# EasyVision-Ton/VMG

Hardware: AMD Instinct MI355X
Metric: LR-frames/s (train: forward+loss+backward+AdamW), VMG-REDS-few_levels 4x SR (higher is better)
Workload: dtype bf16; 1 GPU; VMG-REDS-few_levels train step, per-GPU batch 4x7x3x64x64 -> 4x SR (BASELINE configs[1]); global_batch=4, frames_per_clip=7, parallelism=dp1, launch=eager, recompute_chains=False, fp8_chains=False

## Files before the change

vmg_amd/csrc/ltam.hip:

```cpp
#include "common.h"

namespace {

constexpr int LT_TILE = 8;
constexpr int LT_PIX = 64;
constexpr int LT_HEADS = 4;
constexpr int LT_MAX_T = 32;

struct LtamK {
  const char* q;
  const char* k[LT_MAX_T];
  const char* v[LT_MAX_T];
  const float* loc;
  const float* rpe;
  const float* decay;
  char* out;
  float* lse;
  const char* dout;
  char* dq;
  void* dk_acc[LT_MAX_T];
  void* dv_acc[LT_MAX_T];
  float* drpe;
  int n, h, w, c, t, wh, ww;
  float scale;
  int tiles_x, tiles_y;
  int dbg;
};

__device__ __forceinline__ int nearest_index(float lx, float ly, int w, int h) {
  const float dx = (float)(w - 1 > 1 ? w - 1 : 1), dy = (float)(h - 1 > 1 ? h - 1 : 1);
  const float gx = __fsub_rn(__fdiv_rn(__fmul_rn(2.0f, lx), dx), 1.0f);
  const float gy = __fsub_rn(__fdiv_rn(__fmul_rn(2.0f, ly), dy), 1.0f);
  const float ix = __fmul_rn(__fdiv_rn(__fadd_rn(gx, 1.0f), 2.0f), (float)(w - 1));
  const float iy = __fmul_rn(__fdiv_rn(__fadd_rn(gy, 1.0f), 2.0f), (float)(h - 1));
  const float xn = nearbyintf(ix), yn = nearbyintf(iy);
  if (!(xn >= 0.f && xn <= (float)(w - 1) && yn >= 0.f && yn <= (float)(h - 1))) return -1;
  return (int)yn * w + (int)xn;
}

__device__ __forceinline__ float quad_sum(float v) {
  v += __shfl_xor(v, 1, 64);
  v += __shfl_xor(v, 2, 64);
  return v;
}

typedef __attribute__((ext_vector_type(4))) unsigned int lt_u32x4;
__device__ __attribute__((aligned(16))) unsigned int g_ltam_zero[4] = {0, 0, 0, 0};

template <typename T, int D>
struct RowCopy {
  static constexpr int VN = 16 / sizeof(T), NVEC = LT_HEADS * D / VN, TOTAL = LT_PIX * NVEC, NIT = (TOTAL + 255) / 256;
  lt_u32x4 r[NIT];
  __device__ __forceinline__ void fetch(const T* src_base, const int* src_idx, int tid) {
    constexpr int c = LT_HEADS * D;
#pragma unroll
    for (int k = 0; k < NIT; ++k) {
      const int i = tid + k * 256;
      const int p = min(i / NVEC, LT_PIX - 1), v = i - (i / NVEC) * NVEC;
      const int s_ = src_idx[p];
      const bool ok = i < TOTAL && s_ >= 0;
      const T* src = ok ? src_base + (long long)s_ * c + v * VN : reinterpret_cast<const T*>(g_ltam_zero);
      r[k] = *reinterpret_cast<const lt_u32x4*>(src);
    }
  }
  __device__ __forceinline__ void store(T* dst, int row_stride, int tid) const {
#pragma unroll
    for (int k = 0; k < NIT; ++k) {
      const int i = tid + k * 256;
      const int p = i / NVEC, v = i - p * NVEC;
      if (i < TOTAL) *reinterpret_cast<lt_u32x4*>(dst + p * row_stride + v * VN) = r[k];
    }
  }
};

template <typename T, int D>
__device__ __forceinline__ void load_slice(const T* p, float (&o)[D]) {
  static_assert(D % 4 == 0, "head dim must be a multiple of 4");
  if constexpr (sizeof(T) == 2) {
#pragma unroll
    for (int i = 0; i < D / 4; ++i) {
      const bf16x4 t = *reinterpret_cast<const bf16x4*>(reinterpret_cast<const bf16*>(p) + 4 * i);
#pragma unroll
      for (int e = 0; e < 4; ++e) o[4 * i + e] = (float)t[e];
    }
  } else {
#pragma unroll
    for (int i = 0; i < D / 4; ++i) {
      const f32x4 t = *reinterpret_cast<const f32x4*>(reinterpret_cast<const float*>(p) + 4 * i);
#pragma unroll
      for (int e = 0; e < 4; ++e) o[4 * i + e] = t[e];
    }
  }
}

template <typename T, int D>
__global__ __launch_bounds__(256) void ltam_fwd_kernel(const LtamK a) {
  extern __shared__ __attribute__((aligned(16))) char smem[];
  constexpr int c = LT_HEADS * D, RS = c + 16 / sizeof(T);
  T* qt = reinterpret_cast<T*>(smem);
  T* kt = qt + LT_PIX * RS;
  T* vt = kt + LT_PIX * RS;
  float* knorm = reinterpret_cast<float*>(vt + LT_PIX * RS);
  int* sidx = reinterpret_cast<int*>(knorm + LT_PIX);
  int* selfidx = sidx + LT_PIX;

  const int tid = threadIdx.x, p = tid >> 2, hd = tid & 3;
  const int tyi = p >> 3, txi = p & 7;
  int bid = blockIdx.x;
  const int tx = bid % a.tiles_x;
  bid /= a.tiles_x;
  const int ty = bid % a.tiles_y, n = bid / a.tiles_y;
  const int y = ty * LT_TILE + tyi, x = tx * LT_TILE + txi;
  const bool inside = y < a.h && x < a.w;
  const long long img = (long long)n * a.h * a.w;
  if (tid < LT_PIX) {
    const int yy = ty * LT_TILE + (tid >> 3), xx = tx * LT_TILE + (tid & 7);
    selfidx[tid] = (yy < a.h && xx < a.w) ? yy * a.w + xx : -1;
  }
  __syncthreads();
  RowCopy<T, D> rk, rv;
  rk.fetch(reinterpret_cast<const T*>(a.q) + img * c, selfidx, tid);
  rk.store(qt, RS, tid);
  __syncthreads();
  float qs[D];
  float ss = 0.f;
  load_slice<T, D>(qt + p * RS + hd * D, qs);
#pragma unroll
  for (int d = 0; d < D; ++d) ss += qs[d] * qs[d];
  {
    const float inv = a.scale / fmaxf(sqrtf(quad_sum(ss)), 1e-12f);
#pragma unroll
    for (int d = 0; d < D; ++d) qs[d] *= inv;
  }
  const int wq = a.wh * a.ww;
  const int wy0 = (tyi / a.wh) * a.wh, wx0 = (txi / a.ww) * a.ww;
  const int qi = (tyi - wy0) * a.ww + (txi - wx0);
  const float dec = a.decay[hd];
  float m = -INFINITY, l = 0.f, acc[D];
#pragma unroll
  for (int d = 0; d < D; ++d) acc[d] = 0.f;

  for (int j = 0; j < a.t; ++j) {
    __syncthreads();
    if (tid < LT_PIX) {
      int s = -1;
      if (selfidx[tid] >= 0) {
        const long long lb = ((long long)n * 2 * a.t + 2 * j) * a.h * a.w + selfidx[tid];
        s = nearest_index(a.loc[lb], a.loc[lb + (long long)a.h * a.w], a.w, a.h);
      }
      sidx[tid] = s;
    }
    __syncthreads();
    rk.fetch(reinterpret_cast<const T*>(a.k[j]) + img * c, sidx, tid);
    rv.fetch(reinterpret_cast<const T*>(a.v[j]) + img * c, sidx, tid);
    rk.store(kt, RS, tid);
    rv.store(vt, RS, tid);
    __syncthreads();
    {
      float s2 = 0.f, kv[D];
      load_slice<T, D>(kt + p * RS + hd * D, kv);
#pragma unroll
      for (int d = 0; d < D; ++d) s2 += kv[d] * kv[d];
      s2 = quad_sum(s2);
      if (hd == 0) knorm[p] = fmaxf(sqrtf(s2), 1e-12f);
    }
    __syncthreads();
    float pw = dec;
    for (int e = 1; e < a.t - j; ++e) pw *= dec;
    for (int ki = 0; ki < wq; ++ki) {
      const int pk = (wy0 + ki / a.ww) * LT_TILE + wx0 + ki % a.ww;
      float dot = 0.f, kk[D], vv[D];
      load_slice<T, D>(kt + pk * RS + hd * D, kk);
      load_slice<T, D>(vt + pk * RS + hd * D, vv);
#pragma unroll
      for (int d = 0; d < D; ++d) dot += qs[d] * kk[d];
      const float logit = dot / knorm[pk] + pw * a.rpe[(hd * wq + qi) * wq + ki];
      const float mn = fmaxf(m, logit);
      const float corr = __expf(m - mn), pe = __expf(logit - mn);
      l = l * corr + pe;
#pragma unroll
      for (int d = 0; d < D; ++d) acc[d] = acc[d] * corr + pe * vv[d];
      m = mn;
    }
  }
  if (inside) {
    const float inv = 1.f / l;
    T* o = reinterpret_cast<T*>(a.out) + (img + (long long)y * a.w + x) * c + hd * D;
#pragma unroll
    for (int d = 0; d < D; ++d) o[d] = from_f32<T>(acc[d] * inv);
    if (a.lse) a.lse[(img + (long long)y * a.w + x) * LT_HEADS + hd] = m + __logf(l);
  }
}

template <int C>
__device__ __forceinline__ void scatter_rows(void* acc, long long img, const float* rowbuf, const int* sidx, const int* selfidx, int tid, bool skip) {
  float* dst = reinterpret_cast<float*>(acc);
  for (int i = tid; i < LT_PIX * C; i += 256) {
    const int pp = i / C, ch = i - pp * C;
    const int sp = sidx[pp];
    if (sp >= 0 && selfidx[pp] >= 0 && !skip) atomicAdd(dst + (img + sp) * C + ch, rowbuf[i]);
  }
}

#ifdef VMG_DIAG
#define LT_ABL(bit) (a.dbg & (bit))
#else
#define LT_ABL(bit) false
#endif
template <typename T, int D>
__global__ __launch_bounds__(256) void ltam_bwd_kernel(const LtamK a) {
  extern __shared__ __attribute__((aligned(16))) char smem[];
  constexpr int c = LT_HEADS * D, RS = c + 16 / sizeof(T);
  T* kt = reinterpret_cast<T*>(smem);
  T* vt = kt + LT_PIX * RS;
  T* dot_ = vt + LT_PIX * RS;
  T* qt = dot_ + LT_PIX * RS;
  float* knorm = reinterpret_cast<float*>(qt + LT_PIX * RS);
  float* qnorm = knorm + LT_PIX;
  float* lse = qnorm + LT_PIX;
  float* delta = lse + LT_PIX * LT_HEADS;
  float* drpe_s = delta + LT_PIX * LT_HEADS;
  int* sidx = reinterpret_cast<int*>(drpe_s + LT_HEADS * a.wh * a.ww * a.wh * a.ww);
  int* selfidx = sidx + LT_PIX;

  const int tid = threadIdx.x, p = tid >> 2, hd = tid & 3;
  const int tyi = p >> 3, txi = p & 7;
  int bid = blockIdx.x;
  const int tx = bid % a.tiles_x;
  bid /= a.tiles_x;
  const int ty = bid % a.tiles_y, n = bid / a.tiles_y;
  const int y = ty * LT_TILE + tyi, x = tx * LT_TILE + txi;
  const bool inside = y < a.h && x < a.w;
  const long long img = (long long)n * a.h * a.w;
  const int wq = a.wh * a.ww;
  if (tid < LT_PIX) {
    const int yy = ty * LT_TILE + (tid >> 3), xx = tx * LT_TILE + (tid & 7);
    selfidx[tid] = (yy < a.h && xx < a.w) ? yy * a.w + xx : -1;
  }
  for (int i = tid; i < LT_HEADS * wq * wq; i += 256) drpe_s[i] = 0.f;
  __syncthreads();
  RowCopy<T, D> rk, rv;
  rk.fetch(reinterpret_cast<const T*>(a.dout) + img * c, selfidx, tid);
  rv.fetch(reinterpret_cast<const T*>(a.q) + img * c, selfidx, tid);
  rk.store(dot_, RS, tid);
  rv.store(qt, RS, tid);
  __syncthreads();
  float qn[D], go[D];
  {
    float ss = 0.f, dl = 0.f, ov[D];
    const long long own = (img + (long long)(inside ? y * a.w + x : 0)) * c + hd * D;
    load_slice<T, D>(qt + p * RS + hd * D, qn);
    load_slice<T, D>(dot_ + p * RS + hd * D, go);
    load_slice<T, D>(reinterpret_cast<const T*>(a.out) + own, ov);
#pragma unroll
    for (int d = 0; d < D; ++d) {
      ss += qn[d] * qn[d];
      dl += inside ? go[d] * ov[d] : 0.f;
    }
    const float nr = fmaxf(sqrtf(quad_sum(ss)), 1e-12f);
    if (hd == 0) qnorm[p] = nr;
    const float inv = 1.f / nr;
#pragma unroll
    for (int d = 0; d < D; ++d) qn[d] *= inv;
    delta[p * LT_HEADS + hd] = dl;
    lse[p * LT_HEADS + hd] = inside ? a.lse[(img + (long long)y * a.w + x) * LT_HEADS + hd] : 0.f;
  }
  const int wy0 = (tyi / a.wh) * a.wh, wx0 = (txi / a.ww) * a.ww;
  const int myi = (tyi - wy0) * a.ww + (txi - wx0);
  const float dec = a.decay[hd];
  float dqn[D];
#pragma unroll
  for (int d = 0; d < D; ++d) dqn[d] = 0.f;
  for (int j = 0; j < a.t; ++j) {
    __syncthreads();
    if (tid < LT_PIX) {
      int s = -1;
      if (selfidx[tid] >= 0) {
        const long long lb = ((long long)n * 2 * a.t + 2 * j) * a.h * a.w + selfidx[tid];
        s = nearest_index(a.loc[lb], a.loc[lb + (long long)a.h * a.w], a.w, a.h);
      }
      sidx[tid] = s;
    }
    __syncthreads();
    if (!(LT_ABL(8) && j > 0)) {
      rk.fetch(reinterpret_cast<const T*>(a.k[j]) + img * c, sidx, tid);
      rv.fetch(reinterpret_cast<const T*>(a.v[j]) + img * c, sidx, tid);
    }
    rk.store(kt, RS, tid);
    rv.store(vt, RS, tid);
    __syncthreads();
    float kn[D], vown[D];
    load_slice<T, D>(vt + p * RS + hd * D, vown);
    {
      float s2 = 0.f;
      load_slice<T, D>(kt + p * RS + hd * D, kn);
#pragma unroll
      for (int d = 0; d < D; ++d) s2 += kn[d] * kn[d];
      s2 = quad_sum(s2);
      const float nr = fmaxf(sqrtf(s2), 1e-12f);
      if (hd == 0) knorm[p] = nr;
      const float inv = 1.f / nr;
#pragma unroll
      for (int d = 0; d < D; ++d) kn[d] *= inv;
    }
    __syncthreads();
    float pw = dec;
    for (int e = 1; e < a.t - j; ++e) pw *= dec;

    if (!LT_ABL(4)) {
      const float my_lse = lse[p * LT_HEADS + hd], my_delta = delta[p * LT_HEADS + hd];
      for (int ki = 0; ki < wq; ++ki) {
        const int pk = (wy0 + ki / a.ww) * LT_TILE + wx0 + ki % a.ww;
        const float inv_kn = 1.f / knorm[pk];
        float dot = 0.f, dp = 0.f, kk[D], vv[D];
        load_slice<T, D>(kt + pk * RS + hd * D, kk);
        load_slice<T, D>(vt + pk * RS + hd * D, vv);
#pragma unroll
        for (int d = 0; d < D; ++d) {
          dot += qn[d] * kk[d];
          dp += go[d] * vv[d];
        }
        const float logit = a.scale * dot * inv_kn + pw * a.rpe[(hd * wq + myi) * wq + ki];
        const float pr = __expf(logit - my_lse);
        const float ds = pr * (dp - my_delta);
        if (inside) atomicAdd(&drpe_s[(hd * wq + myi) * wq + ki], ds * pw);
        const float f = ds * a.scale * inv_kn;
#pragma unroll
        for (int d = 0; d < D; ++d) dqn[d] += f * kk[d];
      }
    }
    float dkn[D], dv[D];
#pragma unroll
    for (int d = 0; d < D; ++d) dkn[d] = dv[d] = 0.f;
    for (int qq = 0; qq < wq; ++qq) {
      const int pq = (wy0 + qq / a.ww) * LT_TILE + wx0 + qq % a.ww;
      if (selfidx[pq] < 0 || LT_ABL(2)) continue;
      const float inv_qn = 1.f / qnorm[pq];
      float dot = 0.f, dp = 0.f;
      float qv[D], gg[D];
      load_slice<T, D>(qt + pq * RS + hd * D, qv);
      load_slice<T, D>(dot_ + pq * RS + hd * D, gg);
#pragma unroll
      for (int d = 0; d < D; ++d) {
        qv[d] *= inv_qn;
        dot += qv[d] * kn[d];
        dp += gg[d] * vown[d];
      }
      const float logit = a.scale * dot + pw * a.rpe[(hd * wq + qq) * wq + myi];
      const float pr = __expf(logit - lse[pq * LT_HEADS + hd]);
      const float ds = pr * (dp - delta[pq * LT_HEADS + hd]);
#pragma unroll
      for (int d = 0; d < D; ++d) {
        dkn[d] += ds * a.scale * qv[d];
        dv[d] += pr * gg[d];
      }
    }
    {
      float nd = 0.f;
#pragma unroll
      for (int d = 0; d < D; ++d) nd += kn[d] * dkn[d];
      nd = quad_sum(nd);
      const float inv = 1.f / knorm[p];
      float* rowbuf = reinterpret_cast<float*>(kt);
      __syncthreads();
#pragma unroll
      for (int d = 0; d < D; ++d) rowbuf[p * c + hd * D + d] = (dkn[d] - kn[d] * nd) * inv;
      __syncthreads();
      scatter_rows<c>(a.dk_acc[j], img, rowbuf, sidx, selfidx, tid, LT_ABL(1));
      __syncthreads();
#pragma unroll
      for (int d = 0; d < D; ++d) rowbuf[p * c + hd * D + d] = dv[d];
      __syncthreads();
      scatter_rows<c>(a.dv_acc[j], img, rowbuf, sidx, selfidx, tid, LT_ABL(1));
    }
  }
  {
    float nd = 0.f;
#pragma unroll
    for (int d = 0; d < D; ++d) nd += qn[d] * dqn[d];
    nd = quad_sum(nd);
    if (inside) {
      const float inv = 1.f / qnorm[p];
      T* dq = reinterpret_cast<T*>(a.dq) + (img + (long long)y * a.w + x) * c + hd * D;
#pragma unroll
      for (int d = 0; d < D; ++d) dq[d] = from_f32<T>((dqn[d] - qn[d] * nd) * inv);
    }
  }
  __syncthreads();
  for (int i = tid; i < LT_HEADS * wq * wq; i += 256) atomicAdd(&a.drpe[i], drpe_s[i]);
}

template <typename T, int D>
int launch_ltam(const LtamK& k, bool backward, hipStream_t st) {
  const int RS = k.c + 16 / (int)sizeof(T);
  const int grid = k.n * k.tiles_y * k.tiles_x;
  if (!backward) {
    const int lds = 3 * LT_PIX * RS * (int)sizeof(T) + LT_PIX * 4 + 2 * LT_PIX * 4;
    auto fn = ltam_fwd_kernel<T, D>;
    static bool set[VMG_MAX_DEVICES] = {};
    const int dev = vmg_current_device();
    if (!set[dev]) { (void)hipFuncSetAttribute(reinterpret_cast<const void*>(fn), hipFuncAttributeMaxDynamicSharedMemorySize, 160 * 1024); set[dev] = true; }
    hipLaunchKernelGGL(fn, dim3(grid), dim3(256), lds, st, k);
  } else {
    const int wq = k.wh * k.ww;
    const int lds = 4 * LT_PIX * RS * (int)sizeof(T) + (2 * LT_PIX + 2 * LT_PIX * LT_HEADS + LT_HEADS * wq * wq) * 4 + 2 * LT_PIX * 4;
    VMG_CHECK(lds <= 160 * 1024, "ltam_bwd: LDS request %d B exceeds 160 KiB", lds);
    auto fn = ltam_bwd_kernel<T, D>;
    static bool set[VMG_MAX_DEVICES] = {};
    const int dev = vmg_current_device();
    if (!set[dev]) { (void)hipFuncSetAttribute(reinterpret_cast<const void*>(fn), hipFuncAttributeMaxDynamicSharedMemorySize, 160 * 1024); set[dev] = true; }
    hipLaunchKernelGGL(fn, dim3(grid), dim3(256), lds, st, k);
  }
  VMG_LAUNCH_CHECK();
  return 0;
}

template <typename T>
int dispatch_d(const LtamK& k, bool backward, hipStream_t st) {
  switch (k.c / LT_HEADS) {
    case 4: return launch_ltam<T, 4>(k, backward, st);
    case 8: return launch_ltam<T, 8>(k, backward, st);
    case 28: return launch_ltam<T, 28>(k, backward, st);
    case 36: return launch_ltam<T, 36>(k, backward, st);
  }
  vmg_set_error("ltam: head dim %d not instantiated (supported: 4, 8, 28, 36)", k.c / LT_HEADS);
  return -1;
}

int fill_common(LtamK& k, int dtype, const void* q, const void* const* keys, const void* const* vals, const float* loc, const float* rpe,
                const float* decay, int n, int h, int w, int c, int heads, int wh, int ww, int t, float scale) {
  VMG_CHECK(dtype == VMG_F32 || dtype == VMG_BF16, "ltam: bad dtype");
  VMG_CHECK(q && keys && vals && loc && rpe && decay, "ltam: null pointer");
  VMG_CHECK(heads == LT_HEADS, "ltam: heads must be %d", LT_HEADS);
  VMG_CHECK(t >= 1 && t <= LT_MAX_T, "ltam: 1..%d key-frames", LT_MAX_T);
  VMG_CHECK(n > 0 && h > 0 && w > 0 && c % (LT_HEADS * (dtype == VMG_BF16 ? 8 : 4) / LT_HEADS) == 0 && c % LT_HEADS == 0, "ltam: bad shape");
  VMG_CHECK(wh >= 1 && ww >= 1 && LT_TILE % wh == 0 && LT_TILE % ww == 0 && h % wh == 0 && w % ww == 0 && wh * ww <= 16,
            "ltam: window %dx%d must divide 8 and the image", wh, ww);
  memset(&k, 0, sizeof(k));
  k.q = (const char*)q;
  for (int j = 0; j < t; ++j) {
    VMG_CHECK(keys[j] && vals[j], "ltam: null key/value %d", j);
    k.k[j] = (const char*)keys[j];
    k.v[j] = (const char*)vals[j];
  }
  k.loc = loc; k.rpe = rpe; k.decay = decay;
  k.n = n; k.h = h; k.w = w; k.c = c; k.t = t; k.wh = wh; k.ww = ww; k.scale = scale;
  k.tiles_x = cdiv(w, LT_TILE); k.tiles_y = cdiv(h, LT_TILE);
  return 0;
}

}

extern "C" int vmg_ltam_fwd(int dtype, const void* q, const void* const* keys, const void* const* vals, const float* loc,
                            const float* rpe, const float* decay, void* out, float* lse, int n, int h, int w, int c, int heads, int wh,
                            int ww, int t, float scale, void* stream) {
  LtamK k;
  if (int rc = fill_common(k, dtype, q, keys, vals, loc, rpe, decay, n, h, w, c, heads, wh, ww, t, scale)) return rc;
  VMG_CHECK(out, "ltam_fwd: null output");
  k.out = (char*)out; k.lse = lse;
  return dtype == VMG_BF16 ? dispatch_d<bf16>(k, false, (hipStream_t)stream) : dispatch_d<float>(k, false, (hipStream_t)stream);
}

extern "C" int vmg_ltam_bwd(int dtype, const void* q, const void* const* keys, const void* const* vals, const float* loc,
                            const float* rpe, const float* decay, const void* out, const float* lse, const void* dout, void* dq,
                            void* const* dk_acc, void* const* dv_acc, float* drpe, int n, int h, int w, int c, int heads, int wh,
                            int ww, int t, float scale, void* stream) {
  LtamK k;
  if (int rc = fill_common(k, dtype, q, keys, vals, loc, rpe, decay, n, h, w, c, heads, wh, ww, t, scale)) return rc;
  VMG_CHECK(out && lse && dout && dq && dk_acc && dv_acc && drpe, "ltam_bwd: null pointer");
#ifdef VMG_DIAG
  { const char* e = getenv("VMG_LTAM_DBG"); k.dbg = e ? atoi(e) : 0; }
#endif
  k.out = (char*)out; k.lse = (float*)lse; k.dout = (const char*)dout; k.dq = (char*)dq; k.drpe = drpe;
  for (int j = 0; j < t; ++j) {
    VMG_CHECK(dk_acc[j] && dv_acc[j], "ltam_bwd: null accumulator %d", j);
    k.dk_acc[j] = dk_acc[j];
    k.dv_acc[j] = dv_acc[j];
  }
  return dtype == VMG_BF16 ? dispatch_d<bf16>(k, true, (hipStream_t)stream) : dispatch_d<float>(k, true, (hipStream_t)stream);
}
```

vmg_amd/csrc/warp.hip:

```cpp
#include "common.h"

namespace {

__device__ __forceinline__ float unnorm_coord(float pix, float flow, int size) {
  const float g = __fadd_rn(pix, flow);
  const float denom = (float)(size - 1 > 1 ? size - 1 : 1);
  const float gn = __fsub_rn(__fdiv_rn(__fmul_rn(2.0f, g), denom), 1.0f);
  return __fmul_rn(__fdiv_rn(__fadd_rn(gn, 1.0f), 2.0f), (float)(size - 1));
}

__device__ __forceinline__ float clip_border(float v, int size, float* grad_mult) {
  const float hi = (float)(size - 1);
  if (v <= 0.f) { if (grad_mult) *grad_mult = 0.f; return 0.f; }
  if (v >= hi) { if (grad_mult) *grad_mult = 0.f; return hi; }
  if (grad_mult) *grad_mult = 1.f;
  return v;
}

template <typename T>
struct V16 {
  static constexpr int N = 16 / sizeof(T);
  T v[N];
};

template <typename T>
__global__ __launch_bounds__(256) void warp_bilinear_fwd_kernel(const T* __restrict__ x, const float* __restrict__ flow,
                                                                T* __restrict__ out, int N, int H, int W, int C) {
  constexpr int VN = V16<T>::N;
  const int nvec = C / VN;
  const long long total = (long long)N * H * W * nvec;
  for (long long i = blockIdx.x * 256LL + threadIdx.x; i < total; i += (long long)gridDim.x * 256) {
    const int v = (int)(i % nvec);
    const long long pix = i / nvec;
    const int px = (int)(pix % W);
    const int py = (int)((pix / W) % H);
    const long long n = pix / ((long long)W * H);
    const float fx = flow[pix * 2], fy = flow[pix * 2 + 1];
    const float ix = clip_border(unnorm_coord((float)px, fx, W), W, nullptr);
    const float iy = clip_border(unnorm_coord((float)py, fy, H), H, nullptr);
    const float x0f = floorf(ix), y0f = floorf(iy);
    const int x0 = (int)x0f, y0 = (int)y0f, x1 = x0 + 1, y1 = y0 + 1;
    const float x1f = x0f + 1.f, y1f = y0f + 1.f;
    const float wnw = (x1f - ix) * (y1f - iy), wne = (ix - x0f) * (y1f - iy), wsw = (x1f - ix) * (iy - y0f), wse = (ix - x0f) * (iy - y0f);
    const T* base = x + n * H * W * C + v * VN;
    float acc[VN];
#pragma unroll
    for (int e = 0; e < VN; ++e) acc[e] = 0.f;
    auto corner = [&](int yy, int xx, float wgt) {
      if (yy >= 0 && yy < H && xx >= 0 && xx < W) {
        const V16<T> t = *reinterpret_cast<const V16<T>*>(base + ((long long)yy * W + xx) * C);
#pragma unroll
        for (int e = 0; e < VN; ++e) acc[e] += to_f32(t.v[e]) * wgt;
      }
    };
    corner(y0, x0, wnw);
    corner(y0, x1, wne);
    corner(y1, x0, wsw);
    corner(y1, x1, wse);
    V16<T> o;
#pragma unroll
    for (int e = 0; e < VN; ++e) o.v[e] = from_f32<T>(acc[e]);
    *reinterpret_cast<V16<T>*>(out + pix * C + v * VN) = o;
  }
}

typedef __attribute__((ext_vector_type(2))) __bf16 wp_bf16x2;
template <typename T>
__global__ __launch_bounds__(256) void warp_bilinear_bwd_kernel(const T* __restrict__ x, const float* __restrict__ flow,
                                                                const T* __restrict__ dy, float* __restrict__ dx_acc,
                                                                float* __restrict__ dflow, int N, int H, int W, int C) {
  const int lane = threadIdx.x & 63;
  const long long npix = (long long)N * H * W;
  for (long long pix = blockIdx.x * 4LL + (threadIdx.x >> 6); pix < npix; pix += (long long)gridDim.x * 4) {
    const int px = (int)(pix % W);
    const int py = (int)((pix / W) % H);
    const long long n = pix / ((long long)W * H);
    const float fx = flow[pix * 2], fy = flow[pix * 2 + 1];
    float gmx, gmy;
    const float ix = clip_border(unnorm_coord((float)px, fx, W), W, &gmx);
    const float iy = clip_border(unnorm_coord((float)py, fy, H), H, &gmy);
    const float x0f = floorf(ix), y0f = floorf(iy);
    const int x0 = (int)x0f, y0 = (int)y0f, x1 = x0 + 1, y1 = y0 + 1;
    const float x1f = x0f + 1.f, y1f = y0f + 1.f;
    const float tx = ix - x0f, ty = iy - y0f;
    const float wnw = (x1f - ix) * (y1f - iy), wne = (ix - x0f) * (y1f - iy), wsw = (x1f - ix) * (iy - y0f), wse = (ix - x0f) * (iy - y0f);
    const bool vnw = y0 >= 0 && y0 < H && x0 >= 0 && x0 < W, vne = y0 >= 0 && y0 < H && x1 >= 0 && x1 < W;
    const bool vsw = y1 >= 0 && y1 < H && x0 >= 0 && x0 < W, vse = y1 >= 0 && y1 < H && x1 >= 0 && x1 < W;
    const long long ib = n * H * W * C;
    const long long onw = ib + ((long long)y0 * W + x0) * C, one = ib + ((long long)y0 * W + x1) * C;
    const long long osw = ib + ((long long)y1 * W + x0) * C, ose = ib + ((long long)y1 * W + x1) * C;
    float gix = 0.f, giy = 0.f;
    if constexpr (sizeof(T) == 2) {
      for (int cb = 0; cb < C; cb += 128) {
        const int cp = cb + 2 * lane;
        const bool in = cp < C;
        const long long own = pix * C;
        const int cl = in ? cp : 0;
        const wp_bf16x2 gp = *reinterpret_cast<const wp_bf16x2*>(dy + own + cl);
        const wp_bf16x2 xnw = *reinterpret_cast<const wp_bf16x2*>(x + (vnw ? onw : own) + cl), xne = *reinterpret_cast<const wp_bf16x2*>(x + (vne ? one : own) + cl);
        const wp_bf16x2 xsw = *reinterpret_cast<const wp_bf16x2*>(x + (vsw ? osw : own) + cl), xse = *reinterpret_cast<const wp_bf16x2*>(x + (vse ? ose : own) + cl);
        const float g0 = in ? (float)gp[0] : 0.f, g1 = in ? (float)gp[1] : 0.f;
        const int sl = lane >> 1;
        const float a0 = __shfl(g0, sl, 64), a1 = __shfl(g1, sl, 64), b0 = __shfl(g0, 32 + sl, 64), b1 = __shfl(g1, 32 + sl, 64);
        const float glo = (lane & 1) ? a1 : a0, ghi = (lane & 1) ? b1 : b0;
        const int clo = cb + lane, chi = cb + 64 + lane;
        auto corner = [&](long long o, float wgt, float sx, float sy, wp_bf16x2 xp) __attribute__((always_inline)) {
          if (clo < C) atomicAdd(dx_acc + o + clo, glo * wgt);
          if (chi < C) atomicAdd(dx_acc + o + chi, ghi * wgt);
          const float xv = (float)xp[0] * g0 + (float)xp[1] * g1;
          gix += xv * sx;
          giy += xv * sy;
        };
        if (vnw) corner(onw, wnw, -(1.f - ty), -(1.f - tx), xnw);
        if (vne) corner(one, wne, (1.f - ty), -tx, xne);
        if (vsw) corner(osw, wsw, -ty, (1.f - tx), xsw);
        if (vse) corner(ose, wse, ty, tx, xse);
      }
    } else {
      for (int c = lane; c < C; c += 64) {
        const float g = to_f32(dy[pix * C + c]);
        if (vnw) { atomicAdd(dx_acc + onw + c, g * wnw); const float xv = to_f32(x[onw + c]) * g; gix -= xv * (1.f - ty); giy -= xv * (1.f - tx); }
        if (vne) { atomicAdd(dx_acc + one + c, g * wne); const float xv = to_f32(x[one + c]) * g; gix += xv * (1.f - ty); giy -= xv * tx; }
        if (vsw) { atomicAdd(dx_acc + osw + c, g * wsw); const float xv = to_f32(x[osw + c]) * g; gix -= xv * ty; giy += xv * (1.f - tx); }
        if (vse) { atomicAdd(dx_acc + ose + c, g * wse); const float xv = to_f32(x[ose + c]) * g; gix += xv * ty; giy += xv * tx; }
      }
    }
    gix = wave_sum(gix);
    giy = wave_sum(giy);
    if (lane == 0) {
      dflow[pix * 2] = gix * gmx;
      dflow[pix * 2 + 1] = giy * gmy;
    }
  }
}

__global__ __launch_bounds__(256) void warp_nearest_planes_kernel(const float* __restrict__ loc, const float* __restrict__ flow,
                                                                  float* __restrict__ out, int N, int K2, int H, int W) {
  const long long total = (long long)N * H * W;
  for (long long pix = blockIdx.x * 256LL + threadIdx.x; pix < total; pix += (long long)gridDim.x * 256) {
    const int px = (int)(pix % W);
    const int py = (int)((pix / W) % H);
    const long long n = pix / ((long long)W * H);
    const float ix = clip_border(unnorm_coord((float)px, flow[pix * 2], W), W, nullptr);
    const float iy = clip_border(unnorm_coord((float)py, flow[pix * 2 + 1], H), H, nullptr);
    const int xn = (int)nearbyintf(ix), yn = (int)nearbyintf(iy);
    const bool ok = xn >= 0 && xn < W && yn >= 0 && yn < H;
    for (int k = 0; k < K2; ++k) {
      const long long plane = (n * K2 + k) * H * W;
      out[plane + (long long)py * W + px] = ok ? loc[plane + (long long)yn * W + xn] : 0.f;
    }
  }
}

int grid_for(long long total) {
  long long b = (total + 255) / 256;
  return (int)(b > 8192 ? 8192 : (b < 1 ? 1 : b));
}

__device__ __forceinline__ int fs_reflect(int p, int n) { return p < n ? p : 2 * (n - 1) - p; }

__global__ void flow_smooth_fwd_kernel(const float* __restrict__ in, float* __restrict__ out, long long planes, int H, int W, int r) {
  const long long total = planes * H * W;
  const float inv = 1.0f / (float)(r * r);
  for (long long i = blockIdx.x * (long long)blockDim.x + threadIdx.x; i < total; i += (long long)gridDim.x * blockDim.x) {
    const int x = (int)(i % W), y = (int)((i / W) % H);
    const float* pl = in + (i / ((long long)W * H)) * H * W;
    const int y0 = (y / r) * r, x0 = (x / r) * r;
    float s = 0.f;
    for (int dy = 0; dy < r; ++dy) {
      const float* row = pl + (long long)fs_reflect(y0 + dy, H) * W;
      for (int dx = 0; dx < r; ++dx) s += row[fs_reflect(x0 + dx, W)];
    }
    out[i] = s * inv;
  }
}

__global__ void flow_smooth_bwd_kernel(const float* __restrict__ dout, float* __restrict__ din, long long planes, int H, int W, int r) {
  const long long total = planes * H * W;
  const int hf = (H + r - 1) / r * r, wf = (W + r - 1) / r * r;
  const float inv = 1.0f / (float)(r * r);
  for (long long i = blockIdx.x * (long long)blockDim.x + threadIdx.x; i < total; i += (long long)gridDim.x * blockDim.x) {
    const int x = (int)(i % W), y = (int)((i / W) % H);
    const float* pl = dout + (i / ((long long)W * H)) * H * W;
    int py[2] = {y, 2 * (H - 1) - y}, px[2] = {x, 2 * (W - 1) - x};
    const int ny = (py[1] >= H && py[1] < hf) ? 2 : 1, nx = (px[1] >= W && px[1] < wf) ? 2 : 1;
    float acc = 0.f;
    for (int a = 0; a < ny; ++a) {
      const int y0 = (py[a] / r) * r;
      for (int b = 0; b < nx; ++b) {
        const int x0 = (px[b] / r) * r;
        float g = 0.f;
        for (int dy = 0; dy < r && y0 + dy < H; ++dy)
          for (int dx = 0; dx < r && x0 + dx < W; ++dx) g += pl[(long long)(y0 + dy) * W + x0 + dx];
        acc += g;
      }
    }
    din[i] = acc * inv;
  }
}

}

extern "C" int vmg_warp_bilinear_fwd(int dtype, const void* x, const float* flow, void* out, int N, int H, int W, int C, void* stream) {
  VMG_CHECK(dtype == VMG_F32 || dtype == VMG_BF16, "warp_fwd: bad dtype");
  VMG_CHECK(x && flow && out && N > 0 && H > 0 && W > 0 && C > 0, "warp_fwd: bad arguments");
  const int vn = dtype == VMG_BF16 ? 8 : 4;
  VMG_CHECK(C % vn == 0, "warp_fwd: C must be a multiple of %d", vn);
  VMG_CHECK(((uintptr_t)x | (uintptr_t)out) % 16 == 0, "warp_fwd: pointers must be 16-byte aligned");
  const long long total = (long long)N * H * W * (C / vn);
  hipStream_t st = (hipStream_t)stream;
  if (dtype == VMG_BF16) hipLaunchKernelGGL(warp_bilinear_fwd_kernel<bf16>, dim3(grid_for(total)), dim3(256), 0, st, (const bf16*)x, flow, (bf16*)out, N, H, W, C);
  else hipLaunchKernelGGL(warp_bilinear_fwd_kernel<float>, dim3(grid_for(total)), dim3(256), 0, st, (const float*)x, flow, (float*)out, N, H, W, C);
  VMG_LAUNCH_CHECK();
  return 0;
}

extern "C" int vmg_warp_bilinear_bwd(int dtype, const void* x, const float* flow, const void* dy, void* dx_acc, float* dflow, int N,
                                     int H, int W, int C, void* stream) {
  VMG_CHECK(dtype == VMG_F32 || dtype == VMG_BF16, "warp_bwd: bad dtype");
  VMG_CHECK(x && flow && dy && dx_acc && dflow && N > 0 && H > 0 && W > 0 && C > 0, "warp_bwd: bad arguments");
  const int vn = dtype == VMG_BF16 ? 8 : 4;
  (void)vn;
  const long long total = (long long)N * H * W * 64;
  hipStream_t st = (hipStream_t)stream;
  if (dtype == VMG_BF16) {
    VMG_CHECK(C % 2 == 0 && ((uintptr_t)x | (uintptr_t)dy | (uintptr_t)dx_acc) % 4 == 0, "warp_bwd: bf16 needs an even channel count and 4-byte aligned tensors");
    hipLaunchKernelGGL(warp_bilinear_bwd_kernel<bf16>, dim3(grid_for(total)), dim3(256), 0, st, (const bf16*)x, flow, (const bf16*)dy, (float*)dx_acc, dflow, N, H, W, C);
  } else {
    hipLaunchKernelGGL(warp_bilinear_bwd_kernel<float>, dim3(grid_for(total)), dim3(256), 0, st, (const float*)x, flow, (const float*)dy, (float*)dx_acc, dflow, N, H, W, C);
  }
  VMG_LAUNCH_CHECK();
  return 0;
}

extern "C" int vmg_warp_nearest_planes(const float* loc, const float* flow, float* out, int N, int K2, int H, int W, void* stream) {
  VMG_CHECK(loc && flow && out && N > 0 && K2 > 0 && H > 0 && W > 0, "warp_nearest: bad arguments");
  hipLaunchKernelGGL(warp_nearest_planes_kernel, dim3(grid_for((long long)N * H * W)), dim3(256), 0, (hipStream_t)stream, loc, flow, out, N, K2, H, W);
  VMG_LAUNCH_CHECK();
  return 0;
}

extern "C" int vmg_flow_smooth(const float* in, float* out, int64_t planes, int H, int W, int r, int backward, void* stream) {
  VMG_CHECK(in && out && planes > 0 && H > 0 && W > 0 && r >= 1, "flow_smooth: bad arguments");
  const int hf = (H + r - 1) / r * r, wf = (W + r - 1) / r * r;
  VMG_CHECK(hf - H < H && wf - W < W, "flow_smooth: the reflected padding must be smaller than the plane (as F.pad(mode='reflect') demands)");
  const long long total = planes * H * W;
  if (backward) hipLaunchKernelGGL(flow_smooth_bwd_kernel, dim3(grid_for(total)), dim3(256), 0, (hipStream_t)stream, in, out, (long long)planes, H, W, r);
  else hipLaunchKernelGGL(flow_smooth_fwd_kernel, dim3(grid_for(total)), dim3(256), 0, (hipStream_t)stream, in, out, (long long)planes, H, W, r);
  VMG_LAUNCH_CHECK();
  return 0;
}
```

Baseline: 598.9 LR-frames/s.

## Software-pipeline LTAM backward K/V gathers with double-buffered sample indices

The LTAM backward kernel now double-buffers the per-frame sample-index array and prefetches the loc values and K/V row gathers for frame j+1 while frame j is computed. This hides global-load latency that the loop previously exposed on every frame, and drops one barrier per iteration. The cost is a little more LDS, extra registers for the in-flight fetch, and more subtle index handling. The warp backward kernel also gains diagnostic ablation flags that are compiled out by default.

```diff
diff --git a/vmg_amd/csrc/ltam.hip b/vmg_amd/csrc/ltam.hip
--- a/vmg_amd/csrc/ltam.hip
+++ b/vmg_amd/csrc/ltam.hip
@@ -221,7 +221,7 @@
   float* delta = lse + LT_PIX * LT_HEADS;
   float* drpe_s = delta + LT_PIX * LT_HEADS;
   int* sidx = reinterpret_cast<int*>(drpe_s + LT_HEADS * a.wh * a.ww * a.wh * a.ww);
-  int* selfidx = sidx + LT_PIX;
+  int* selfidx = sidx + 2 * LT_PIX;
 
   const int tid = threadIdx.x, p = tid >> 2, hd = tid & 3;
   const int tyi = p >> 3, txi = p & 7;
@@ -271,24 +271,35 @@
   float dqn[D];
 #pragma unroll
   for (int d = 0; d < D; ++d) dqn[d] = 0.f;
+  float lxn = 0.f, lyn = 0.f;
+  auto loc_load = [&](int j) __attribute__((always_inline)) {
+    if (tid < LT_PIX && selfidx[tid] >= 0) {
+      const long long lb = ((long long)n * 2 * a.t + 2 * j) * a.h * a.w + selfidx[tid];
+      lxn = a.loc[lb];
+      lyn = a.loc[lb + (long long)a.h * a.w];
+    }
+  };
+  auto sidx_put = [&](int j) __attribute__((always_inline)) {
+    if (tid < LT_PIX) sidx[(j & 1) * LT_PIX + tid] = selfidx[tid] >= 0 ? nearest_index(lxn, lyn, a.w, a.h) : -1;
+  };
+  loc_load(0);
+  sidx_put(0);
+  if (a.t > 1) loc_load(1);
+  __syncthreads();
+  rk.fetch(reinterpret_cast<const T*>(a.k[0]) + img * c, sidx, tid);
+  rv.fetch(reinterpret_cast<const T*>(a.v[0]) + img * c, sidx, tid);
   for (int j = 0; j < a.t; ++j) {
-    __syncthreads();
-    if (tid < LT_PIX) {
-      int s = -1;
-      if (selfidx[tid] >= 0) {
-        const long long lb = ((long long)n * 2 * a.t + 2 * j) * a.h * a.w + selfidx[tid];
-        s = nearest_index(a.loc[lb], a.loc[lb + (long long)a.h * a.w], a.w, a.h);
-      }
-      sidx[tid] = s;
-    }
-    __syncthreads();
-    if (!(LT_ABL(8) && j > 0)) {
-      rk.fetch(reinterpret_cast<const T*>(a.k[j]) + img * c, sidx, tid);
-      rv.fetch(reinterpret_cast<const T*>(a.v[j]) + img * c, sidx, tid);
-    }
+    const int* sj = sidx + (j & 1) * LT_PIX;
+    __syncthreads();
     rk.store(kt, RS, tid);
     rv.store(vt, RS, tid);
-    __syncthreads();
+    if (j + 1 < a.t) sidx_put(j + 1);
+    if (j + 2 < a.t) loc_load(j + 2);
+    __syncthreads();
+    if (j + 1 < a.t && !LT_ABL(8)) {
+      rk.fetch(reinterpret_cast<const T*>(a.k[j + 1]) + img * c, sidx + ((j + 1) & 1) * LT_PIX, tid);
+      rv.fetch(reinterpret_cast<const T*>(a.v[j + 1]) + img * c, sidx + ((j + 1) & 1) * LT_PIX, tid);
+    }
     float kn[D], vown[D];
     load_slice<T, D>(vt + p * RS + hd * D, vown);
     {
@@ -366,12 +377,12 @@
 #pragma unroll
       for (int d = 0; d < D; ++d) rowbuf[p * c + hd * D + d] = (dkn[d] - kn[d] * nd) * inv;
       __syncthreads();
-      scatter_rows<c>(a.dk_acc[j], img, rowbuf, sidx, selfidx, tid, LT_ABL(1));
+      scatter_rows<c>(a.dk_acc[j], img, rowbuf, sj, selfidx, tid, LT_ABL(1));
       __syncthreads();
 #pragma unroll
       for (int d = 0; d < D; ++d) rowbuf[p * c + hd * D + d] = dv[d];
       __syncthreads();
-      scatter_rows<c>(a.dv_acc[j], img, rowbuf, sidx, selfidx, tid, LT_ABL(1));
+      scatter_rows<c>(a.dv_acc[j], img, rowbuf, sj, selfidx, tid, LT_ABL(1));
     }
   }
   {
@@ -403,7 +414,7 @@
     hipLaunchKernelGGL(fn, dim3(grid), dim3(256), lds, st, k);
   } else {
     const int wq = k.wh * k.ww;
-    const int lds = 4 * LT_PIX * RS * (int)sizeof(T) + (2 * LT_PIX + 2 * LT_PIX * LT_HEADS + LT_HEADS * wq * wq) * 4 + 2 * LT_PIX * 4;
+    const int lds = 4 * LT_PIX * RS * (int)sizeof(T) + (2 * LT_PIX + 2 * LT_PIX * LT_HEADS + LT_HEADS * wq * wq) * 4 + 3 * LT_PIX * 4;
     VMG_CHECK(lds <= 160 * 1024, "ltam_bwd: LDS request %d B exceeds 160 KiB", lds);
     auto fn = ltam_bwd_kernel<T, D>;
     static bool set[VMG_MAX_DEVICES] = {};
diff --git a/vmg_amd/csrc/warp.hip b/vmg_amd/csrc/warp.hip
--- a/vmg_amd/csrc/warp.hip
+++ b/vmg_amd/csrc/warp.hip
@@ -65,10 +65,16 @@
 }
 
 typedef __attribute__((ext_vector_type(2))) __bf16 wp_bf16x2;
+#ifdef VMG_DIAG
+#define WP_ABL(bit) (dbg & (bit))
+#else
+#define WP_ABL(bit) false
+#endif
 template <typename T>
 __global__ __launch_bounds__(256) void warp_bilinear_bwd_kernel(const T* __restrict__ x, const float* __restrict__ flow,
                                                                 const T* __restrict__ dy, float* __restrict__ dx_acc,
-                                                                float* __restrict__ dflow, int N, int H, int W, int C) {
+                                                                float* __restrict__ dflow, int N, int H, int W, int C, int dbg) {
+  (void)dbg;
   const int lane = threadIdx.x & 63;
   const long long npix = (long long)N * H * W;
   for (long long pix = blockIdx.x * 4LL + (threadIdx.x >> 6); pix < npix; pix += (long long)gridDim.x * 4) {
@@ -97,16 +103,16 @@
         const long long own = pix * C;
         const int cl = in ? cp : 0;
         const wp_bf16x2 gp = *reinterpret_cast<const wp_bf16x2*>(dy + own + cl);
-        const wp_bf16x2 xnw = *reinterpret_cast<const wp_bf16x2*>(x + (vnw ? onw : own) + cl), xne = *reinterpret_cast<const wp_bf16x2*>(x + (vne ? one : own) + cl);
-        const wp_bf16x2 xsw = *reinterpret_cast<const wp_bf16x2*>(x + (vsw ? osw : own) + cl), xse = *reinterpret_cast<const wp_bf16x2*>(x + (vse ? ose : own) + cl);
+        const wp_bf16x2 xnw = *reinterpret_cast<const wp_bf16x2*>(x + (vnw && !WP_ABL(2) ? onw : own) + cl), xne = *reinterpret_cast<const wp_bf16x2*>(x + (vne && !WP_ABL(2) ? one : own) + cl);
+        const wp_bf16x2 xsw = *reinterpret_cast<const wp_bf16x2*>(x + (vsw && !WP_ABL(2) ? osw : own) + cl), xse = *reinterpret_cast<const wp_bf16x2*>(x + (vse && !WP_ABL(2) ? ose : own) + cl);
         const float g0 = in ? (float)gp[0] : 0.f, g1 = in ? (float)gp[1] : 0.f;
         const int sl = lane >> 1;
         const float a0 = __shfl(g0, sl, 64), a1 = __shfl(g1, sl, 64), b0 = __shfl(g0, 32 + sl, 64), b1 = __shfl(g1, 32 + sl, 64);
         const float glo = (lane & 1) ? a1 : a0, ghi = (lane & 1) ? b1 : b0;
         const int clo = cb + lane, chi = cb + 64 + lane;
         auto corner = [&](long long o, float wgt, float sx, float sy, wp_bf16x2 xp) __attribute__((always_inline)) {
-          if (clo < C) atomicAdd(dx_acc + o + clo, glo * wgt);
-          if (chi < C) atomicAdd(dx_acc + o + chi, ghi * wgt);
+          if (clo < C && !WP_ABL(1)) atomicAdd(dx_acc + o + clo, glo * wgt);
+          if (chi < C && !WP_ABL(1)) atomicAdd(dx_acc + o + chi, ghi * wgt);
           const float xv = (float)xp[0] * g0 + (float)xp[1] * g1;
           gix += xv * sx;
           giy += xv * sy;
@@ -219,15 +225,17 @@
                                      int H, int W, int C, void* stream) {
   VMG_CHECK(dtype == VMG_F32 || dtype == VMG_BF16, "warp_bwd: bad dtype");
   VMG_CHECK(x && flow && dy && dx_acc && dflow && N > 0 && H > 0 && W > 0 && C > 0, "warp_bwd: bad arguments");
-  const int vn = dtype == VMG_BF16 ? 8 : 4;
-  (void)vn;
+  int dbg = 0;
+#ifdef VMG_DIAG
+  { const char* e = getenv("VMG_WARP_DBG"); dbg = e ? atoi(e) : 0; }
+#endif
   const long long total = (long long)N * H * W * 64;
   hipStream_t st = (hipStream_t)stream;
   if (dtype == VMG_BF16) {
     VMG_CHECK(C % 2 == 0 && ((uintptr_t)x | (uintptr_t)dy | (uintptr_t)dx_acc) % 4 == 0, "warp_bwd: bf16 needs an even channel count and 4-byte aligned tensors");
-    hipLaunchKernelGGL(warp_bilinear_bwd_kernel<bf16>, dim3(grid_for(total)), dim3(256), 0, st, (const bf16*)x, flow, (const bf16*)dy, (float*)dx_acc, dflow, N, H, W, C);
+    hipLaunchKernelGGL(warp_bilinear_bwd_kernel<bf16>, dim3(grid_for(total)), dim3(256), 0, st, (const bf16*)x, flow, (const bf16*)dy, (float*)dx_acc, dflow, N, H, W, C, dbg);
   } else {
-    hipLaunchKernelGGL(warp_bilinear_bwd_kernel<float>, dim3(grid_for(total)), dim3(256), 0, st, (const float*)x, flow, (const float*)dy, (float*)dx_acc, dflow, N, H, W, C);
+    hipLaunchKernelGGL(warp_bilinear_bwd_kernel<float>, dim3(grid_for(total)), dim3(256), 0, st, (const float*)x, flow, (const float*)dy, (float*)dx_acc, dflow, N, H, W, C, dbg);
   }
   VMG_LAUNCH_CHECK();
   return 0;
```

New measurement: 599.1 LR-frames/s, median of 2. About the same (+0.0%).
